# robotseu/ORB_Line_SLAM

Measured on AMD Instinct MI355X. Metric: stereo frames/s extract+match (ORB+LBD), KITTI 1242x375, higher is better.
Workload: dtype u8; 1 GPU; C3: 1242x375 stereo, 2000 ORB + 500 LBD per image, extract + stereo point/line match + f2f LBD match + SearchByBoW vs the previous frame (synthetic k=10 L=6 vocabulary, ComputeBoW included); parallelism=frame-sharded x1, distinct_pairs=512, order=shuffled, scene=default

## Files before the change

### include/orbline.h

```cpp
#ifndef ORBLINE_H
#define ORBLINE_H

#include "orbline_types.h"

#ifdef __cplusplus
extern "C" {
#endif

typedef struct olf_ctx olf_ctx;

const char* olf_last_error(void);
int olf_device_count(void);
int olf_default_params(olf_params* p);

int  olf_ctx_create(const olf_params* p, int width, int height, int max_images, olf_ctx** out);
void olf_ctx_destroy(olf_ctx* ctx);
int  olf_ctx_synchronize(olf_ctx* ctx);
int  olf_ctx_set_input_event(olf_ctx* ctx, void* hip_event);
int  olf_ctx_set_deferred_join(olf_ctx* ctx, int on);
int  olf_stereo_frames_join_dev(olf_ctx* ctx, void* stream);
int  olf_ctx_poll_status(olf_ctx* ctx);

int olf_profile_enable(olf_ctx* ctx, int on);
int olf_profile_reset(olf_ctx* ctx);
// ... 1 lines not shown
const char* olf_profile_stage_name(int stage);
int olf_profile_read(olf_ctx* ctx, double* total_ms, int32_t* calls);

enum { OLF_RGB2GRAY = 0, OLF_BGR2GRAY = 1, OLF_RGBA2GRAY = 2, OLF_BGRA2GRAY = 3 };
int olf_cvt_gray_dev(olf_ctx* ctx, const uint8_t* d_src, int code, int n_images, uint8_t* d_gray, void* stream);
int olf_remap_linear_dev(olf_ctx* ctx, const uint8_t* d_src, int src_w, int src_h, const float* d_mapx, const float* d_mapy, int dst_w,
                         int dst_h, int n_images, uint8_t* d_dst, void* stream);
int olf_init_undistort_rectify_map_dev(olf_ctx* ctx, const double* K, const double* D, int n_dist, const double* R, const double* P, int w, int h,
                                       float* d_map1, float* d_map2, void* stream);
int olf_init_undistort_rectify_map(olf_ctx* ctx, const double* K, const double* D, int n_dist, const double* R, const double* P, int w, int h,
                                   float* map1, float* map2);
int olf_cvt_gray(olf_ctx* ctx, const uint8_t* src, int code, int n_images, uint8_t* gray);
int olf_remap_linear(olf_ctx* ctx, const uint8_t* src, int src_w, int src_h, const float* mapx, const float* mapy, int dst_w, int dst_h,
                     int n_images, uint8_t* dst);

int olf_distinctive_descriptors(olf_ctx* ctx, const uint8_t* desc, const int32_t* offs, int n_points, int32_t* best);

size_t olf_kf_record_bytes(int n_keys, int n_lines);
int olf_kf_record_pack(uint64_t frame_id, uint64_t kf_id, double timestamp, const float* t3, const float* quat4, int n_keys,
                       const olf_keypoint* keys, const float* uright, const float* depth, const uint8_t* desc, const uint64_t* mappoint_ids,
                       int n_lines, const olf_keyline* lines, const float* disparity2, const double* le3, const uint8_t* ldesc,
                       const uint64_t* mapline_ids, uint8_t* out, size_t capacity, size_t* written);
int olf_kf_record_counts(const uint8_t* buf, size_t len, int32_t* n_keys, int32_t* n_lines, size_t* record_bytes);
int olf_kf_record_unpack(const uint8_t* buf, size_t len, uint64_t* frame_id, uint64_t* kf_id, double* timestamp, float* t3, float* quat4,
                         olf_keypoint* keys, float* uright, float* depth, uint8_t* desc, uint64_t* mappoint_ids, olf_keyline* lines,
                         float* disparity2, double* le3, uint8_t* ldesc, uint64_t* mapline_ids);

typedef struct olf_voc olf_voc;
int olf_voc_create(int k, int L, int scoring, int weighting, int n_nodes, const int32_t* parent, const uint8_t* is_leaf, const uint8_t* desc,
                   const double* weight, olf_voc** out);
int olf_voc_load_text(const char* path, olf_voc** out);
void olf_voc_destroy(olf_voc* voc);
int olf_voc_info(const olf_voc* voc, int* k, int* L, int* scoring, int* weighting, int* n_nodes, int* n_words);
int olf_bow_words_dev(olf_ctx* ctx, const olf_voc* voc, const uint8_t* d_desc, int n, int levelsup, int32_t* d_word, double* d_weight,
                      int32_t* d_node, void* stream);
int olf_bow_assemble(const olf_voc* voc, const int32_t* word, const double* weight, const int32_t* node, int n, int32_t* bow_ids,
                     double* bow_vals, int* n_bow, int32_t* fv_nodes, int32_t* fv_offs, int32_t* fv_idx, int* n_fv);
int olf_bow_transform(olf_ctx* ctx, const olf_voc* voc, const uint8_t* desc, int n, int levelsup, int32_t* bow_ids, double* bow_vals,
                      int* n_bow, int32_t* fv_nodes, int32_t* fv_offs, int32_t* fv_idx, int* n_fv);
int olf_search_by_bow_batch_dev(olf_ctx* ctx, const olf_voc* voc, int n_frames, int img_stride, const olf_keypoint* d_kps, const uint8_t* d_desc,
                                const int32_t* d_counts, const uint8_t* d_mp_valid, const uint8_t* d_mp_bad, float nnratio, int check_orientation,
                                int levelsup, int32_t* d_matches, int32_t* d_nmatches, void* stream);

int olf_orb_scale_tables(const olf_ctx* ctx, float* scale, float* inv_scale, float* sigma2, float* inv_sigma2,
                         int32_t* features_per_level);
int olf_orb_level_sizes(const olf_ctx* ctx, int32_t* widths, int32_t* heights);
int olf_orb_capacity(const olf_ctx* ctx);
int olf_orb_extract_strided(olf_ctx* ctx, const uint8_t* image, size_t row_stride, olf_keypoint* kps, uint8_t* desc, int32_t* count);
int olf_orb_extract_dev(olf_ctx* ctx, const uint8_t* d_images, int n_images, olf_keypoint* d_kps, uint8_t* d_desc,
                        int32_t* d_counts, void* stream);
int olf_orb_extract(olf_ctx* ctx, const uint8_t* images, int n_images, olf_keypoint* kps, uint8_t* desc, int32_t* counts);
int olf_orb_pyramid_level(olf_ctx* ctx, int image, int level, int blurred, uint8_t* dst);
int olf_orb_debug_candidates(olf_ctx* ctx, int image, int level, int32_t* xys, int cap, int32_t* count);
int olf_debug_status(olf_ctx* ctx, int32_t* out64);
int olf_debug_status_n(olf_ctx* ctx, int32_t* out, int n);
int olf_debug_lsd_owner(olf_ctx* ctx, int image, uint32_t* out);
int olf_debug_lsd_regions(olf_ctx* ctx, int image, int32_t* start_n, double* angle, int cap, int32_t* count);
int olf_debug_lsd_waves(olf_ctx* ctx, int waves_per_image, int rob_entries);
int olf_debug_lsd_groups(olf_ctx* ctx, int groups);
int olf_debug_lsd_scatter(olf_ctx* ctx, int on);
int olf_debug_lsd_log_cap(olf_ctx* ctx, int entries);
int olf_debug_seed_sort(olf_ctx* ctx, const uint32_t* keys, int n, int kthr, int depth_limit, uint32_t* out, int32_t* out_n);
int olf_debug_seed_sort_mode(olf_ctx* ctx, int mode);
int olf_debug_seed_sort_wide(olf_ctx* ctx, const uint64_t* keys, int n, int64_t kthr, int depth_limit, int full, uint32_t* out, int32_t* out_n);
int olf_debug_lsd_pool(olf_ctx* ctx, int pool_chunks);
int olf_debug_fdiv_sweep(olf_ctx* ctx, uint64_t seed, int blocks, int per_thread, uint64_t* mismatches);
int olf_debug_sqrtq_sweep(olf_ctx* ctx, int count, uint64_t* mismatches);
int olf_debug_align_sweep(olf_ctx* ctx, uint64_t seed, int blocks, int per_thread, uint64_t* out3);

int olf_stereo_points_dev(olf_ctx* ctx, int n_pairs, const olf_keypoint* d_kps, const uint8_t* d_desc, const int32_t* d_counts,
                          float* d_uright, float* d_depth, void* stream);
int olf_stereo_points(olf_ctx* ctx, const uint8_t* images, int n_pairs, olf_keypoint* kps, uint8_t* desc, int32_t* counts,
                      float* uright, float* depth);

int olf_match_bf_dev(olf_ctx* ctx, const uint8_t* d_descA, const int32_t* d_nA, int strideA, int a_step, const uint8_t* d_descB,
                     const int32_t* d_nB, int strideB, int b_step, int n_sets, float nnr, int best_lr, int32_t* d_m12, void* stream);
int olf_match_bf(olf_ctx* ctx, const uint8_t* descA, int nA, const uint8_t* descB, int nB, float nnr, int best_lr, int32_t* m12);
int olf_knn2(olf_ctx* ctx, const uint8_t* descQ, int nQ, const uint8_t* descT, int nT, int32_t* idx0, int32_t* dist0, int32_t* dist1);
int olf_match_candidates_dev(olf_ctx* ctx, const uint8_t* d_descQ, int nQ, const uint8_t* d_descT, int nT, const int32_t* d_cand_offsets,
                             const int32_t* d_cand_idx, uint16_t* d_dist, void* stream);
int olf_match_candidates(olf_ctx* ctx, const uint8_t* descQ, int nQ, const uint8_t* descT, int nT, const int32_t* cand_offsets,
                         const int32_t* cand_idx, uint16_t* dist);
typedef struct olf_frame_view {
    const olf_keypoint* keys;
    const uint8_t* desc;
    const float*   uright;
    int32_t        n;
    uint8_t*       mp_valid;
    uint8_t*       mp_obs;
    const uint8_t* mp_bad;
    const float*   mp_world;
    const uint8_t* mp_desc;
    const uint8_t* outlier;
    const float*   Tcw;
    float fx, fy, cx, cy, mbf, minX, maxX, minY, maxY;
    const float*   scale_factors;
    int32_t        n_levels;
    const float*   mp_maxd;
    const float*   mp_mind;
    const int32_t* fv_nodes;
    const int32_t* fv_offsets;
    const int32_t* fv_features;
    int32_t        fv_n;
    const int32_t* grid_offsets;
    const int32_t* grid_index;
} olf_frame_view;
// ... 534 lines not shown
```

### orb_line_slam_amd/csrc/api.cpp

```cpp
#include "ctx.hpp"
#include "staging.hpp"
#include <map>
#include <mutex>

namespace olf {
static thread_local std::string g_err;
void set_error(const std::string& s) { g_err = s; }

int check_device(const olf_ctx* c, const char* who)
{
    int d = -1;
    if (hipGetDevice(&d) != hipSuccess || d != c->device) { set_error(std::string(who) + ": the context belongs to another device than the current one"); return OLF_ERR_INVALID; }
    return OLF_OK;
}

static int check_landscape(const olf_ctx* c, const char* who)
{
    if (c->orb.portrait) {
        set_error(std::string(who) + ": the context's image is portrait (a pyramid level's octree would have round(width / height) == 0 root cells, where the "
                                     "reference divides by zero): no detector runs in it");
        return OLF_ERR_INVALID;
    }
    return OLF_OK;
}
// ... 178 lines not shown
    if (c->has_tables) angle_tables_release(c->device, c->params.line.conv_libm_float);
    if (c->h_outslab) (void)hipHostFree(c->h_outslab);
    for (void* p : c->allocs) (void)hipFree(p);
    for (void* p : c->scratch) if (p) (void)hipFree(p);
    for (auto& r : c->prof_recs) { (void)hipEventDestroy(r.a); (void)hipEventDestroy(r.b); }
    for (hipEvent_t e : c->prof_pool) (void)hipEventDestroy(e);
    if (c->ev_fork) (void)hipEventDestroy(c->ev_fork);
    if (c->ev_front) (void)hipEventDestroy(c->ev_front);
    if (c->ev_sort) (void)hipEventDestroy(c->ev_sort);
    if (c->ev_lbd) (void)hipEventDestroy(c->ev_lbd);
    if (c->ev_join) (void)hipEventDestroy(c->ev_join);
    if (c->stream2) (void)hipStreamDestroy(c->stream2);
    if (c->stream) (void)hipStreamDestroy(c->stream);
    delete c;
}

int olf_ctx_create(const olf_params* p, int width, int height, int max_images, olf_ctx** out)
{
    if (!p || !out || width < 64 || height < 64 || max_images < 1) { set_error("olf_ctx_create: bad argument"); return OLF_ERR_INVALID; }
    *out = nullptr;
    if (p->abi_version != OLF_ABI_VERSION || p->struct_size != (uint32_t)sizeof(olf_params)) {
        set_error("olf_ctx_create: the parameter block was not initialised by this library's olf_default_params() (abi_version / struct_size differ: "
                  "caller built against another include/orbline_types.h)");
        return OLF_ERR_INVALID;
    }
    int ndev = 0;
    if (hipGetDeviceCount(&ndev) != hipSuccess || ndev < 1) {
        set_error("olf_ctx_create: no HIP device visible (this library has no CPU path)");
        return OLF_ERR_NODEVICE;
    }
    olf_ctx* c = new olf_ctx();
    c->params = *p; c->W = width; c->H = height; c->max_images = max_images;
    int rc = c->orb.build(p->orb, width, height);
    if (rc != OLF_OK) {
        set_error(rc == OLF_ERR_CAPACITY ? "olf_ctx_create: more than 32760 key points on one pyramid level (nfeatures too large for this scale factor / level count)"
                  : (width > kMaxOrbSide || height > kMaxOrbSide) ? "olf_ctx_create: image wider or higher than 4131 pixels (FAST candidates are packed with 12 bits per coordinate)"
                                         : "olf_ctx_create: image size / ORB parameters not supported (every pyramid level needs at least 62 x 62 pixels)");
        delete c; return rc;
    }
    auto fail = [&](int code) { olf_ctx_destroy(c); return code; };
    if (hipGetDevice(&c->device) != hipSuccess) return fail(OLF_ERR_HIP);
    if (hipDeviceGetAttribute(&c->limits.nCU, hipDeviceAttributeMultiprocessorCount, c->device) != hipSuccess || c->limits.nCU <= 0) c->limits.nCU = 64;
    if (hipDeviceGetAttribute(&c->limits.maxLds, hipDeviceAttributeMaxSharedMemoryPerBlock, c->device) != hipSuccess) c->limits.maxLds = 64 * 1024;
    if (hipStreamCreateWithFlags(&c->stream, hipStreamNonBlocking) != hipSuccess) { set_error("hipStreamCreate failed"); return fail(OLF_ERR_HIP); }
    const OrbGeom& g = c->orb.geom;
    const size_t n = (size_t)max_images;
    OrbDeviceBufs& b = c->ob;
    const bool allocTrace = getenv("OLF_ALLOC_TRACE") != nullptr;
#define A(ptr, count) do { if ((rc = dev_alloc(c, &(ptr), (count))) != OLF_OK) return fail(rc); \
                           if (allocTrace) fprintf(stderr, "alloc %-18s %8.3f MB per image\n", #ptr, (double)(count) * sizeof(*(ptr)) / 1e6 / (double)n); } while (0)
    A(b.pyr, n * g.pyrBytes); A(b.blur, n * g.pyrBytes);
    A(b.cells, n * g.totalCells * g.cellCap); A(b.cellCount, n * g.totalCells);
    A(b.cand, n * g.candTotal); A(b.candNode, n * g.candTotal); A(b.candCount, n * g.nlevels);
    if (g.maxNodes > 2048) A(b.octSpill, n * g.nlevels * octree_lds_bytes(g.maxNodes));
    A(b.lvlKp, n * g.kpTotal); A(b.lvlCount, n * g.nlevels); A(b.lvlAngle, n * g.kpTotal);
    A(b.rx, c->orb.rx.size() + 1); A(b.ry, c->orb.ry.size() + 1); A(b.geom, 1); A(b.status, 256);
    A(c->d_sad, ((n + 1) / 2) * g.outCap); A(c->d_bestkey, ((n + 1) / 2) * g.outCap); A(c->d_rowperm, n * g.outCap);
    A(c->d_images, n * width * height);
#undef A
    if (hipMemcpy(b.rx, c->orb.rx.data(), c->orb.rx.size() * sizeof(ResizeCoef), hipMemcpyHostToDevice) != hipSuccess ||
        hipMemcpy(b.ry, c->orb.ry.data(), c->orb.ry.size() * sizeof(ResizeCoef), hipMemcpyHostToDevice) != hipSuccess ||
        hipMemcpy(b.geom, &g, sizeof(OrbGeom), hipMemcpyHostToDevice) != hipSuccess ||
        hipMemset(b.status, 0, 1024) != hipSuccess) {
        set_error("olf_ctx_create: table upload failed");
        return fail(OLF_ERR_HIP);
    }
    rc = c->line.build(p->line, width, height, max_images);
    if (rc != OLF_OK) { set_error("olf_ctx_create: LSD parameters not supported"); return fail(rc); }
    LineGeom& lg = c->line.geom;
    int prLeast = 0, prGreatest = 0;
    (void)hipDeviceGetStreamPriorityRange(&prLeast, &prGreatest);
    if (hipStreamCreateWithPriority(&c->stream2, hipStreamNonBlocking, prLeast) != hipSuccess ||
        hipEventCreateWithFlags(&c->ev_fork, hipEventDisableTiming) != hipSuccess || hipEventCreateWithFlags(&c->ev_front, hipEventDisableTiming) != hipSuccess || hipEventCreateWithFlags(&c->ev_sort, hipEventDisableTiming) != hipSuccess ||
        hipEventCreateWithFlags(&c->ev_lbd, hipEventDisableTiming) != hipSuccess ||
        hipEventCreateWithFlags(&c->ev_join, hipEventDisableTiming) != hipSuccess) { set_error("stream/event creation failed"); return fail(OLF_ERR_HIP); }
    LineDeviceBufs& l = c->lb;
#define A(ptr, count) do { if ((rc = dev_alloc(c, &(ptr), (count))) != OLF_OK) return fail(rc); \
                           if (allocTrace) fprintf(stderr, "alloc %-18s %8.3f MB per image\n", #ptr, (double)(count) * sizeof(*(ptr)) / 1e6 / (double)n); } while (0)
    const bool batchCtx = n > (size_t)kBatchCtxImages;
    const size_t keyWords = lg.wide ? 2 : 1;
    A(l.grad, n * lg.Ps); A(l.keysA, n * lg.Ps * keyWords); A(l.keysB, n * lg.Ps * keyWords);
    if (batchCtx && lg.Ps * 4 >= lg.pitchW * lg.H && lg.Ps * 4 >= lg.pitchS * lg.Hs) { l.lsdBlur = reinterpret_cast<uint8_t*>(l.keysA); l.scaled = reinterpret_cast<uint8_t*>(l.keysB); c->scaled_aliased = true; }
    else { A(l.lsdBlur, n * lg.pitchW * lg.H); A(l.scaled, n * lg.pitchS * lg.Hs); }
    A(l.topBuf, n * (size_t)lsd_seedsort_top_words()); A(l.keyCount, n * 32); A(l.maxN, n * 32); A(l.chunkCnt, n * ((lg.Ps + 4095) / 4096)); A(l.sortHist, n * (size_t)lsd_sort_max_chunks(lg.Ps) * 32); A(l.sortBase, n * 32);
    l.nChunks = lg.regionStride / 32;
    A(l.region, n * (size_t)lg.regionStride); l.ownerImages = (batchCtx || lg.wide) ? 0 : (int)std::min<size_t>(n, kMwMaxImages); A(l.owner, (size_t)l.ownerImages * lg.Ps); A(l.links, n * (size_t)l.nChunks);
    lg.logCap = lg.regionStride / 2;
    lg.spillBlocks = lg.regionStride / 2 >= lg.Ps ? 0 : (int)std::max<size_t>(4, n / 16);
    if (lg.spillBlocks) A(lg.spillArena, (size_t)lg.spillBlocks * 2 * lg.Ps);
    A(lg.spillCtl, 64); A(lg.spillOf, n);
    l.mgImages = (int)std::min<size_t>(n, kMgMaxImages); l.mgStride = lsd_grow_mg_stride(lg.maxRegions);
    A(l.mg, (size_t)l.mgImages * l.mgStride);
    A(l.rawLines, n * lg.maxDetect); A(l.rawCount, n); A(l.regCount, n); A(l.growFmt, n); A(l.lbdBlur, n * lg.pitchW * lg.H); A(l.dxdy, n * lg.pitchD * lg.H);
    A(l.rowSums, n * lg.outCap * 63 * 4); A(l.lbdStarts, n * lg.outCap * 64 * 2); A(l.rx, c->line.rx.size()); A(l.ry, c->line.ry.size()); A(l.geom, 1);
    A(c->d_ldist, ((n + 1) / 2) * lg.outCap * lg.outCap); A(c->d_lm21, ((n + 1) / 2) * lg.outCap);
    if (hipMalloc(&c->d_lprep, stereo_lines_prep_bytes((int)n, lg.outCap)) != hipSuccess) { set_error("hipMalloc failed"); return fail(OLF_ERR_HIP); }
    c->allocs.push_back(c->d_lprep);
    const bool slab = n <= 16;
    if (slab) {
        size_t off = 0;
        for (int k = 0; k < FB_FIELDS; ++k) { c->outslab_off[k] = off; off += (fb_bytes(c, k, n) + 255) & ~(size_t)255; }
        c->outslab_bytes = off;
        A(c->d_outslab, off);
        if (hipHostMalloc(reinterpret_cast<void**>(&c->h_outslab), off, hipHostMallocDefault) != hipSuccess) { set_error("hipHostMalloc failed"); return fail(OLF_ERR_HIP); }
    }
    for (int k = 0; k < FB_FIELDS; ++k) {
        uint8_t* q = nullptr;
// ... 397 lines not shown
```

### orb_line_slam_amd/csrc/api_debug.cpp

```cpp
#include "ctx.hpp"
#include "staging.hpp"
#include "wg_state.hpp"

namespace olf {
int launch_copy16(const void* src, void* dst, size_t bytes, hipStream_t s);
}

using namespace olf;

static int sweep_counters(HostCall& h, unsigned long long** st, int n)
{
    h.add(st, n);
    OLF_TRY(h.bind(SCRATCH_STAGE));
    OLF_HIP_CHECK(hipMemsetAsync(*st, 0, (size_t)n * 8, h.stream()));
    return OLF_OK;
}

extern "C" {

int olf_orb_pyramid_level(olf_ctx* c, int image, int level, int blurred, uint8_t* dst)
{
    if (!c || !dst || image < 0 || image >= c->max_images || level < 0 || level >= c->orb.geom.nlevels) return OLF_ERR_INVALID;
    const LevelGeom& L = c->orb.geom.lv[level];
    const uint8_t* src = (blurred ? c->ob.blur : c->ob.pyr) + (size_t)image * c->orb.geom.pyrBytes + L.offset;
    OLF_HIP_CHECK(hipStreamSynchronize(c->stream));
    OLF_HIP_CHECK(hipMemcpy2D(dst, L.w, src, L.pitch, L.w, L.h, hipMemcpyDeviceToHost));
    return OLF_OK;
}

int olf_debug_sim3_solver_lds_limit(int bytes)
{
    g_sim3_solver_lds.set(bytes);
    return OLF_OK;
}

int olf_debug_pnp_solver_lds_limit(int bytes)
{
    g_pnp_solver_lds.set(bytes);
    return OLF_OK;
}

int olf_debug_initializer_lds_limit(int bytes)
{
    g_initializer_lds.set(bytes);
    return OLF_OK;
}

int olf_debug_pose_points_lds_limit(int bytes)
{
    g_pose_points_lds.set(bytes);
    return OLF_OK;
}

int olf_debug_optimize_sim3_lds_limit(int bytes)
{
    g_optimize_sim3_lds.set(bytes);
    return OLF_OK;
}

int olf_debug_status(olf_ctx* c, int32_t* out64)
{
    if (!c || !out64) return OLF_ERR_INVALID;
    OLF_HIP_CHECK(hipDeviceSynchronize());
    OLF_HIP_CHECK(hipMemcpy(out64, c->ob.status, 256, hipMemcpyDeviceToHost));
    return OLF_OK;
}

int olf_debug_copy_bandwidth(olf_ctx* c, size_t bytes, int reps, double* gbytes_per_s)
{
    if (!c || !gbytes_per_s || bytes < 16 || reps < 1) { set_error("olf_debug_copy_bandwidth: bad argument"); return OLF_ERR_INVALID; }
    OLF_TRY(check_device(c, "olf_debug_copy_bandwidth"));
    void *a = nullptr, *b = nullptr;
    OLF_HIP_CHECK(hipMalloc(&a, bytes));
    if (hipMalloc(&b, bytes) != hipSuccess) { (void)hipFree(a); set_error("olf_debug_copy_bandwidth: hipMalloc failed"); return OLF_ERR_HIP; }
    hipEvent_t e0, e1;
    (void)hipEventCreate(&e0); (void)hipEventCreate(&e1);
    (void)hipMemsetAsync(a, 1, bytes, c->stream);
    int rc = olf::launch_copy16(a, b, bytes, c->stream);
    (void)hipEventRecord(e0, c->stream);
    for (int i = 0; i < reps && rc == OLF_OK; ++i) rc = olf::launch_copy16(i & 1 ? b : a, i & 1 ? a : b, bytes, c->stream);
// ... 189 lines not shown
```

### orb_line_slam_amd/csrc/host_tables.cpp

```cpp
#include "olf_internal.hpp"
#include "line_internal.hpp"
#include <algorithm>
#include <cmath>
#include <cfenv>

namespace olf {

static inline int cv_round_f(float v) { return (int)lrintf(v); }
static inline int cv_round_d(double v) { return (int)lrint(v); }
static inline int cv_floor(double v) { int i = (int)v; return i - (i > v); }
static inline int cv_ceil(double v) { int i = (int)v; return i + (i < v); }

std::vector<int> gaussian_taps_q8(int n, double sigma, int sum256)
{
    if (sum256) {
        std::vector<double> k(n);
        double s = 0;
        const double scale2X = -0.5 / (sigma * sigma);
        for (int i = 0; i < n; ++i) { const double x = i - (n - 1) * 0.5; k[i] = std::exp(scale2X * x * x); s += k[i]; }
        std::vector<int> q(n);
        double err = 0;
        int sum = 0;
        for (int i = 0; i < n / 2; ++i) {
            const double adj = k[i] / s * 256.0 + err;
// ... 108 lines not shown
        L.offset = off;
        off += L.pitch * L.h;
        off = (off + 255) & ~255;
        L.maxBorderX = L.w - kMinBorder; L.maxBorderY = L.h - kMinBorder;
        const float width = (float)(L.maxBorderX - kMinBorder), height = (float)(L.maxBorderY - kMinBorder);
        L.nCols = (int)(width / 30.f); L.nRows = (int)(height / 30.f);
        L.wCell = (int)std::ceil(width / L.nCols); L.hCell = (int)std::ceil(height / L.nRows);
        L.wCellM = (uint32_t)(((1u << 20) + L.wCell - 1) / L.wCell); L.hCellM = (uint32_t)(((1u << 20) + L.hCell - 1) / L.hCell);
        if (L.w >= (1 << 14) || L.h >= (1 << 14) || L.wCell > 64 || L.hCell > 64) { L.wCellM = 0; L.hCellM = 0; }
        L.cellBase = cells;
        cells += L.nCols * L.nRows;
        cellCap = std::max(cellCap, ((L.wCell + 1) / 2) * ((L.hCell + 1) / 2));
        L.quota = nPerLevel[l];
        maxQuota = std::max(maxQuota, L.quota);
        L.nIni = (int)std::round(width / height);
        if (L.nIni < 1) { portrait = true; L.nIni = 1; }
        L.hX = width / L.nIni;
        L.scale = sf[l]; L.inv_scale = inv_sf[l];
        L.patch_size = (int)(31 * sf[l]);
        L.kpBase = kps; L.kpCap = std::max(L.quota + 8, 4 * L.nIni + 4); kps += L.kpCap;
        maxKp = std::max(maxKp, L.kpCap);
        if (l > 0) {
            const LevelGeom& P = g.lv[l - 1];
            L.resizeTabX = (int)rx.size(); L.resizeTabY = (int)ry.size();
            rx.resize(rx.size() + L.w); ry.resize(ry.size() + L.h);
            double inv_x = (double)L.w / P.w, inv_y = (double)L.h / P.h;
            resize_axis_coefs(P.w, L.w, 1. / inv_x, true, &rx[L.resizeTabX]);
            resize_axis_coefs(P.h, L.h, 1. / inv_y, false, &ry[L.resizeTabY]);
            L.resizeTiled = resize_tiled_fits(&rx[L.resizeTabX], &ry[L.resizeTabY], P.w, P.h, L.w, L.h) ? 1 : 0;
            if (L.resizeTiled && resize_strip_fits(&rx[L.resizeTabX], P.w, L.w)) L.resizeTiled |= 2;
        }
    }
    g.pyrBytes = off;
    g.totalCells = cells;
    g.cellCap = cellCap;
    if (cellCap > 1024) return OLF_ERR_CAPACITY;
    for (int l = 0; l < nlevels; ++l) {
        LevelGeom& L = g.lv[l];
        long cap = (long)L.nCols * L.nRows * cellCap;
        L.candCap = (int)std::min<long>(cap, 65535);
        L.candBase = cand;
        cand += (L.candCap + 63) & ~63;
    }
    g.candTotal = cand;
    g.kpTotal = kps;
    g.outCap = kps;
    int mn = 64;
    while (mn < maxKp) mn <<= 1;
    g.maxNodes = mn;
    if (mn > 32768) return OLF_ERR_CAPACITY;
    return OLF_OK;
}

int LineHostTables::build(const olf_line_params& p, int W, int H, int max_images)
{
    LineGeom& g = geom;
    g = LineGeom();
    if (p.lsd_refine < 0 || p.lsd_refine > 2) return OLF_ERR_INVALID;
    if (p.conv_seed_order != 0 && p.conv_seed_order != 1) return OLF_ERR_INVALID;
    if (p.conv_libm_float != 0 && p.conv_libm_float != 1) return OLF_ERR_INVALID;
    if (!(p.lsd_scale > 0) || p.lsd_n_bins < 2 || p.lsd_n_bins > (1 << 24) || !(p.lsd_ang_th > 0 && p.lsd_ang_th < 180)) return OLF_ERR_INVALID;
    const double kPI = 3.1415926535897932384626433832795;
    g.W = W; g.H = H; g.pitchW = (W + 63) & ~63; g.pitchD = (W + 3) & ~3;
    g.scale = p.lsd_scale;
    g.Ws = cv_round_d(W * p.lsd_scale); g.Hs = cv_round_d(H * p.lsd_scale);
    g.pitchS = (g.Ws + 63) & ~63;
    g.Ps = g.Ws * g.Hs;
    {
        int k = 0; while ((1 << k) < g.Ws) ++k;
        const int p = std::max(32, 22 + k);
        const unsigned long long M = ((1ull << p) + (unsigned long long)g.Ws - 1) / (unsigned long long)g.Ws;
        g.divWsM = (uint32_t)M; g.divWsS = p - 32;
    }
    g.libmFloat = p.conv_libm_float ? 1 : 0;
    g.alignDeg = p.lsd_ang_th < 90 ? (float)(180.0 - p.lsd_ang_th) : -1.f;
    g.regionStride = std::max(1024 + g.Ps / 32 + 64, (2 * g.Ps + 31) / 32) * 32;
    if (max_images > kBatchCtxImages) g.regionStride = ((std::max(g.Ps, 8192) + 31) / 32) * 32;
    if ((long)g.Ws * g.Hs >= (1L << 27) || g.Ws < 8 || g.Hs < 8 || g.Ws > 32767 || g.Hs > 32767) return OLF_ERR_INVALID;
    g.wide = (p.lsd_n_bins > 1024 || (long)g.Ws * g.Hs >= (1L << 22)) ? 1 : 0;
    g.prec = kPI * p.lsd_ang_th / 180;
    {
        const long double w = (long double)(2 * kPI) - (long double)g.prec;
        double t = (double)w;
        if ((long double)t < w) t = std::nextafter(t, 1e300);
        g.precWrap = t;
    }
    {
        const double m = 6e-4;
        if (p.lsd_ang_th <= 80.0) {
            g.alignTanLo = std::nextafter((float)std::tan(g.prec - m), 0.f);
            g.alignTanHi = std::nextafter((float)std::tan(g.prec + m), 1e30f);
        } else { g.alignTanLo = -1.f; g.alignTanHi = -1.f; }
    }
    const double pp = p.lsd_ang_th / 180;
    const double rho = p.lsd_quant / std::sin(g.prec);
    int n = 0;
    while (!(std::sqrt(n / 4.0) > rho)) ++n;
    g.nThr = n;
    g.nBins = p.lsd_n_bins;
    const double LOG_NT = 5 * (std::log10(double(g.Ws)) + std::log10(double(g.Hs))) / 2 + std::log10(11.0);
    g.minRegSize = int(-LOG_NT / std::log10(pp));
    g.logNT = LOG_NT; g.logEps = p.lsd_log_eps; g.pProb = pp;
    g.minLength = p.min_line_length * std::min(W, H);
    g.maxDetect = std::min(32768, std::max(4096, g.Ps / 48));
    if (p.lsd_nfeatures == 0) g.maxDetect = std::min(g.maxDetect, std::max(4096, (int)(16e9 / ((double)std::max(max_images, 1) * 63 * 16))));
    g.maxRegions = std::min(g.Ps / std::max(g.minRegSize, 1) + 1, g.Ps / 6 - 1);
// ... 51 lines not shown
```

### orb_line_slam_amd/csrc/olf_internal.hpp

```cpp
#pragma once
#include <hip/hip_runtime.h>
#include <stdint.h>
#include <string>
#include <vector>
#include "../../include/orbline_types.h"
#include "device_math.hpp"

#define OLF_HIP_CHECK(expr)                                                                 \
    do {                                                                                    \
        hipError_t _e = (expr);                                                             \
        if (_e != hipSuccess) {                                                             \
            olf::set_error(std::string(#expr) + ": " + hipGetErrorString(_e));              \
            return OLF_ERR_HIP;                                                             \
        }                                                                                   \
    } while (0)

#define OLF_TRY(expr)                  \
    do {                               \
        int _rc = (expr);              \
        if (_rc != OLF_OK) return _rc; \
    } while (0)

struct olf_ctx;

// ... 108 lines not shown
};

struct ResizeCoef { int16_t ofs; int16_t a0; int16_t a1; int16_t pad; };

struct OrbGeom {
    int nlevels;
    int W, H, in_pitch;
    int pyrBytes;
    int totalCells;
    int cellCap;
    int candTotal;
    int kpTotal;
    int outCap;
    int iniTh, minTh;
    int maxNodes;
    LevelGeom lv[OLF_MAX_LEVELS];
    int umax[16];
    int blurTaps[7];
};

struct OrbHostTables {
    std::vector<float> sf, inv_sf, sigma2, inv_sigma2;
    std::vector<int> nPerLevel;
    OrbGeom geom;
    std::vector<ResizeCoef> rx, ry;
    bool portrait = false;
    int build(const olf_orb_params& p, int W, int H);
};

std::vector<int> gaussian_taps_q8(int n, double sigma, int sum256 = 0);
void resize_axis_coefs(int sn, int dn, double scale, bool clamp_like_x, ResizeCoef* coef);

struct OrbDeviceBufs {
    uint8_t* pyr = nullptr;
    uint8_t* blur = nullptr;
    uint32_t* cells = nullptr;
    int* cellCount = nullptr;
    uint32_t* cand = nullptr;
    uint16_t* candNode = nullptr;
    int* candCount = nullptr;
    uint32_t* lvlKp = nullptr;
    int* lvlCount = nullptr;
    float* lvlAngle = nullptr;
    ResizeCoef* rx = nullptr;
    ResizeCoef* ry = nullptr;
    OrbGeom* geom = nullptr;
    int* status = nullptr;
    unsigned char* octSpill = nullptr;
};

int launch_orb_pyramid(const OrbGeom& g, const OrbDeviceBufs& b, const uint8_t* d_in, int n_images, hipStream_t s);
int launch_orb_fast(const OrbGeom& g, const OrbDeviceBufs& b, int n_images, hipStream_t s);
int launch_orb_octree(const OrbGeom& g, const OrbDeviceBufs& b, int n_images, hipStream_t s);
size_t octree_lds_bytes(int M);
int launch_orb_blur(const OrbGeom& g, const OrbDeviceBufs& b, int n_images, hipStream_t s);
int launch_orb_describe(const OrbGeom& g, const OrbDeviceBufs& b, int n_images, olf_keypoint* d_kps, uint8_t* d_desc,
                        int* d_counts, int out_cap, hipStream_t s);

struct Taps7 { int t[7]; };
int launch_sep7(const uint8_t* src, size_t srcImgStride, int srcPitch, uint8_t* dst, size_t dstImgStride, int dstPitch, int W, int H,
                const int* taps7, int n_images, hipStream_t s);
int launch_sep_wide(const uint8_t* src, size_t srcImgStride, int srcPitch, uint8_t* dst, size_t dstImgStride, int dstPitch, int W, int H,
                    const int* taps, int r, int n_images, hipStream_t s);

bool resize_tiled_fits(const ResizeCoef* rx, const ResizeCoef* ry, int sw, int sh, int dw, int dh);
bool resize_strip_fits(const ResizeCoef* rx, int sw, int dw, int ncols = 4);
int launch_resize_tiled(const uint8_t* src, size_t srcImgStride, int srcPitch, int sw, int sh, uint8_t* dst, size_t dstImgStride, int dstPitch,
                        int dw, int dh, const ResizeCoef* d_rx, const ResizeCoef* d_ry, int n_images, hipStream_t s, bool strip = false);

int launch_cvt_gray(const uint8_t* src, uint8_t* dst, int w, int h, int code, int n_images, hipStream_t s);
int launch_init_rectify_map(const double* ir9, const double* k8, double fx, double fy, double u0, double v0, int w, int h, float* d_map1, float* d_map2,
                            hipStream_t s);
int launch_remap_linear(const uint8_t* src, int sw, int sh, const float* mapx, const float* mapy, int dw, int dh, uint8_t* dst, int n_images,
                        hipStream_t s);

int launch_stereo_points(const OrbGeom& g, const OrbDeviceBufs& b, int n_pairs, const olf_keypoint* d_kps, const uint8_t* d_desc,
                         const int* d_counts, int cap, float mbf, float fx, float* d_uRight, float* d_depth, int* d_sad, int* d_bestKey,
                         unsigned* d_perm, hipStream_t s);
int launch_match_bf(const uint8_t* dA, const int* nA, int strideA, int aStep, const uint8_t* dB, const int* nB, int strideB, int bStep,
                    int n_sets, float nnr, int best_lr, int* ws, int* m12, hipStream_t s);
int launch_knn2(const uint8_t* dA, const int* nA, int strideA, const uint8_t* dB, const int* nB, int strideB, int n_sets, int* idx0,
                int* dist0, int* dist1, hipStream_t s);
int launch_knn2_indexed(const uint8_t* q, const int* rank_entry, const int* qidx, const int* qbase, const int* nQ, const int* tile_prefix, int n_sets,
                        int max_tiles, const uint8_t* t, const int* nT, int strideT, int tStep, int tCap, int* idx0, int* dist0, int* dist1, hipStream_t s);
int launch_match_candidates(const uint8_t* q, int nQ, const uint8_t* t, int nT, const int* offs, const int* cand, uint16_t* out, hipStream_t s);
int launch_distinctive(const uint8_t* desc, const int* offs, int n_points, int* best, hipStream_t s);
int launch_hamming_matrix(const uint8_t* a, int nA, const uint8_t* b, int nB, uint16_t* out, hipStream_t s);


inline bool grid_scales(float minX, float maxX, float minY, float maxY, float* wInv, float* hInv)
{
    if (!(maxX > minX) || !(maxY > minY)) return false;
    *wInv = static_cast<float>(OLF_GRID_COLS) / (maxX - minX);
    *hInv = static_cast<float>(OLF_GRID_ROWS) / (maxY - minY);
    return true;
}
int launch_assign_grid(const olf_keypoint* d_kps, size_t frame_stride, const int* d_counts, int count_stride, int n_fixed, int n_limit, float minX,
                       float minY, float wInv, float hInv, int n_frames, int* d_cell_offsets, int* d_cell_index, size_t index_stride, hipStream_t s);
int launch_features_in_area(const olf_keypoint* d_keys, const int* d_cell_offsets, const int* d_cell_index, float minX, float minY, float wInv, float hInv,
                            int n_queries, const olf_area_query* d_queries, int* d_cand_offsets, int* d_cand_idx, int cand_capacity, int* d_status,
                            hipStream_t s);
bool grid_is_valid(const int32_t* cell_offsets, const int32_t* cell_index, int n);

int launch_kfdb_tables(const int* d_qoff, const int* d_qids, const double* d_qvals, int n_queries, const int* d_beg, const int* d_len, const int* d_ids,
                       const double* d_vals, int n_slots, int* d_common, int* d_first, double* d_score, hipStream_t s);
int launch_bow_score_pairs(const int* d_pairs, int n_pairs, const int* a_beg, const int* a_len, int n_a, const int* a_ids, const double* a_vals,
                           const int* b_beg, const int* b_len, int n_b, const int* b_ids, const double* b_vals, double* d_score, hipStream_t s);
// ... 3 lines not shown
```

### orb_line_slam_amd/csrc/orb_octree.hip

```cpp
#include "olf_internal.hpp"

namespace olf {

struct NodeRec { short ulx, uly, urx, bry; };

__device__ __forceinline__ int wave_incl_scan(int v, int lane)
{
#pragma unroll
    for (int o = 1; o < 64; o <<= 1) {
        int t = __shfl_up(v, o);
        if (lane >= o) v += t;
    }
    return v;
}

__device__ int block_excl_scan(int* a, int n, int* wsum)
{
    const int tid = threadIdx.x, lane = tid & 63, wv = tid >> 6;
    const int chunk = (n + 255) >> 8;
    const int b = tid * chunk, e = min(b + chunk, n);
    int s = 0;
    for (int i = b; i < e; ++i) s += a[i];
    int inc = wave_incl_scan(s, lane);
    if (lane == 63) wsum[wv] = inc;
    __syncthreads();
    int base = 0;
    for (int k = 0; k < wv; ++k) base += wsum[k];
    const int total = wsum[0] + wsum[1] + wsum[2] + wsum[3];
    int run = base + inc - s;
    for (int i = b; i < e; ++i) { int v = a[i]; a[i] = run; run += v; }
    __syncthreads();
    return total;
}

__device__ __forceinline__ int quadrant(const NodeRec& n, int x, int y, int& hx, int& hy)
{
    hx = (int)ceilf((float)(n.urx - n.ulx) / 2);
    hy = (int)ceilf((float)(n.bry - n.uly) / 2);
    return (x < n.ulx + hx ? 0 : 1) + (y < n.uly + hy ? 0 : 2);
}

template <bool SPILL>
__global__ __launch_bounds__(256) void k_octree(const OrbGeom* __restrict__ gp, const uint32_t* __restrict__ cells,
                                                const int* __restrict__ cellCount, uint32_t* __restrict__ cand,
                                                uint16_t* __restrict__ candNode, int* __restrict__ candCount,
                                                uint32_t* __restrict__ lvlKp, int* __restrict__ lvlCount, int* __restrict__ status,
                                                unsigned char* __restrict__ spill, size_t spillBytes)
{
    extern __shared__ __align__(16) unsigned char lds_smem[];
    unsigned char* smem = SPILL ? spill + ((size_t)blockIdx.y * gridDim.x + blockIdx.x) * spillBytes : lds_smem;
    const OrbGeom& g = *gp;
    const int level = blockIdx.x, img = blockIdx.y, tid = threadIdx.x;
    const LevelGeom& L = g.lv[level];
    const int M = g.maxNodes;
    NodeRec* nodeA = reinterpret_cast<NodeRec*>(smem);
    NodeRec* nodeB = nodeA + M;
    int* cntA = reinterpret_cast<int*>(nodeB + M);
    int* cntB = cntA + M;
    int* childCnt = cntB + M;
    int* scanA = childCnt + 4 * M;
    int* scanB = scanA + M;
    int* scanC = scanB + M;
    uint32_t* sortKey = reinterpret_cast<uint32_t*>(scanC + M);
    unsigned short* seqA = reinterpret_cast<unsigned short*>(sortKey + M);
    unsigned short* seqB = seqA + M;
    unsigned short* procNode = seqB + M;
    unsigned short* rankOf = procNode + M;
    unsigned short* seqToNode = rankOf + M;
    int* cellScan = reinterpret_cast<int*>(seqToNode + M);
    __shared__ int wsum[4];
    __shared__ int sh[8];

    const int nCells = L.nCols * L.nRows;
    const int* cc = cellCount + (size_t)img * g.totalCells + L.cellBase;
    uint32_t* myCand = cand + (size_t)img * g.candTotal + L.candBase;
    uint16_t* myNode = candNode + (size_t)img * g.candTotal + L.candBase;

    int C = 0;
    for (int base = 0; base < nCells; base += 4096) {
        const int n = min(4096, nCells - base);
        for (int i = tid; i < n; i += 256) cellScan[i] = cc[base + i];
        __syncthreads();
        const int tot = block_excl_scan(cellScan, n, wsum);
        for (int i = tid; i < n; i += 256) {
            const int k = cc[base + i], o = C + cellScan[i];
            const uint32_t* slot = cells + ((size_t)img * g.totalCells + L.cellBase + base + i) * g.cellCap;
            for (int j = 0; j < k; ++j)
                if (o + j < L.candCap) myCand[o + j] = slot[j];
        }
        C += tot;
        __syncthreads();
    }
    if (C > L.candCap) { if (tid == 0) atomicOr(status, 1); C = L.candCap; }
    if (tid == 0) candCount[img * g.nlevels + level] = C;
    __syncthreads();
    __threadfence_block();

    const int N = L.quota;
    const int nIni = L.nIni;
    for (int i = tid; i < 4 * M; i += 256) childCnt[i] = 0;
    __syncthreads();
    for (int c = tid; c < C; c += 256) {
        const int x = myCand[c] >> 20;
        int r = (int)((float)x / L.hX);
        r = min(r, nIni - 1);
        myNode[c] = (unsigned short)r;
        atomicAdd(&childCnt[r], 1);
    }
    __syncthreads();
    for (int i = tid; i < M; i += 256) scanA[i] = (i < nIni && childCnt[i] > 0) ? 1 : 0;
    __syncthreads();
    int Lsz = block_excl_scan(scanA, nIni, wsum);
    for (int i = tid; i < nIni; i += 256)
        if (childCnt[i] > 0) {
            const int p = scanA[i];
            NodeRec n;
            n.ulx = (short)(int)(L.hX * (float)i); n.urx = (short)(int)(L.hX * (float)(i + 1));
            n.uly = 0; n.bry = (short)(L.maxBorderY - kMinBorder);
            nodeA[p] = n; cntA[p] = childCnt[i]; seqA[p] = (unsigned short)p;
            scanB[i] = p;
        }
    __syncthreads();
    for (int c = tid; c < C; c += 256) myNode[c] = (unsigned short)scanB[myNode[c]];
    __syncthreads();

    NodeRec* cur = nodeA; NodeRec* nxt = nodeB;
    int* curCnt = cntA; int* nxtCnt = cntB;
    unsigned short* curSeq = seqA; unsigned short* nxtSeq = seqB;
    bool careful = false, finish = (C == 0);
    int guard = 0;
    while (!finish && guard++ < 64) {
        for (int i = tid; i < 4 * Lsz; i += 256) childCnt[i] = 0;
        __syncthreads();
        for (int c0 = tid; c0 < C; c0 += 4 * 256) {
            int ni[4];
            uint32_t pp[4];
#pragma unroll
            for (int u = 0; u < 4; ++u) { const int c = c0 + 256 * u; ni[u] = c < C ? (int)myNode[c] : -1; pp[u] = c < C ? myCand[c] : 0u; }
#pragma unroll
            for (int u = 0; u < 4; ++u) {
                const int i = ni[u];
                if (i >= 0 && curCnt[i] > 1) {
                    int hx, hy;
                    const int q = quadrant(cur[i], (int)(pp[u] >> 20), (int)((pp[u] >> 8) & 0xfff), hx, hy);
                    atomicAdd(&childCnt[4 * i + q], 1);
                }
            }
        }
        __syncthreads();
        int E;
        if (!careful) {
            for (int i = tid; i < Lsz; i += 256) scanA[i] = curCnt[i] > 1 ? 1 : 0;
            __syncthreads();
            E = block_excl_scan(scanA, Lsz, wsum);
            for (int i = tid; i < Lsz; i += 256)
                if (curCnt[i] > 1) procNode[scanA[i]] = (unsigned short)i;
        } else {
            for (int i = tid; i < M; i += 256) {
                uint32_t k = 0;
                if (i < Lsz && curCnt[i] > 1) {
                    k = ((uint32_t)min(curCnt[i], 0xffff) << 16) | curSeq[i];
                    seqToNode[curSeq[i]] = (unsigned short)i;
                }
                sortKey[i] = k;
            }
            __syncthreads();
            for (int k = 2; k <= M; k <<= 1)
                for (int j = k >> 1; j > 0; j >>= 1) {
                    for (int i = tid; i < M; i += 256) {
                        const int ixj = i ^ j;
                        if (ixj > i) {
                            const uint32_t a = sortKey[i], b = sortKey[ixj];
                            const bool desc = (i & k) == 0;
                            if (desc ? (a < b) : (a > b)) { sortKey[i] = b; sortKey[ixj] = a; }
                        }
                    }
                    __syncthreads();
                }
            if (tid == 0) sh[0] = 0;
            __syncthreads();
            int cntE = 0;
            for (int i = tid; i < M; i += 256)
                if (sortKey[i] != 0) { procNode[i] = seqToNode[sortKey[i] & 0xffff]; ++cntE; }
            atomicAdd(&sh[0], cntE);
            __syncthreads();
            E = sh[0];
        }
        __syncthreads();
        for (int r = tid; r < E; r += 256) {
            const int i = procNode[r];
            scanB[r] = (childCnt[4 * i] > 0) + (childCnt[4 * i + 1] > 0) + (childCnt[4 * i + 2] > 0) + (childCnt[4 * i + 3] > 0);
        }
        __syncthreads();
        block_excl_scan(scanB, E, wsum);
        if (tid == 0) sh[1] = E;
        __syncthreads();
        if (careful) {
            for (int r = tid; r < E; r += 256) {
                const int i = procNode[r];
                const int nc = (childCnt[4 * i] > 0) + (childCnt[4 * i + 1] > 0) + (childCnt[4 * i + 2] > 0) + (childCnt[4 * i + 3] > 0);
                if (Lsz - (r + 1) + scanB[r] + nc >= N) atomicMin(&sh[1], r + 1);
            }
            __syncthreads();
        }
        const int K = sh[1];
        for (int i = tid; i < Lsz; i += 256) rankOf[i] = 0xffff;
        __syncthreads();
        for (int r = tid; r < K; r += 256) rankOf[procNode[r]] = (unsigned short)r;
        if (tid == 0) {
            int T = 0;
            if (K > 0) {
                const int i = procNode[K - 1];
                T = scanB[K - 1] + (childCnt[4 * i] > 0) + (childCnt[4 * i + 1] > 0) + (childCnt[4 * i + 2] > 0) + (childCnt[4 * i + 3] > 0);
            }
            sh[2] = T; sh[3] = 0;
        }
        __syncthreads();
        const int T = sh[2];
        for (int i = tid; i < Lsz; i += 256) scanC[i] = rankOf[i] == 0xffff ? 1 : 0;
        __syncthreads();
        block_excl_scan(scanC, Lsz, wsum);
        const int newL = T + (Lsz - K);
        int nExp = 0;
        for (int i = tid; i < Lsz; i += 256) {
            const int r = rankOf[i];
            if (r == 0xffff) {
                const int p = T + scanC[i];
                nxt[p] = cur[i]; nxtCnt[p] = curCnt[i]; nxtSeq[p] = 0;
            } else {
                const NodeRec n = cur[i];
                int hx, hy;
                quadrant(n, 0, 0, hx, hy);
                const int c0 = childCnt[4 * i], c1 = childCnt[4 * i + 1], c2 = childCnt[4 * i + 2], c3 = childCnt[4 * i + 3];
                const int nc = (c0 > 0) + (c1 > 0) + (c2 > 0) + (c3 > 0);
                const int base = T - (scanB[r] + nc);
// ... 3 lines not shown
                for (int q = 0; q < 4; ++q) {
                    if (cs[q] > 0) {
                        --after;
                        const int p = base + after;
                        NodeRec ch;
                        ch.ulx = (short)((q & 1) ? n.ulx + hx : n.ulx);
                        ch.urx = (short)((q & 1) ? n.urx : n.ulx + hx);
                        ch.uly = (short)((q & 2) ? n.uly + hy : n.uly);
                        ch.bry = (short)((q & 2) ? n.bry : n.uly + hy);
                        nxt[p] = ch; nxtCnt[p] = cs[q];
                        nxtSeq[p] = (unsigned short)(scanB[r] + before);
                        ++before;
                        if (cs[q] > 1) ++nExp;
                        childCnt[4 * i + q] = p + 1;
                    }
                }
            }
        }
        atomicAdd(&sh[3], nExp);
        __syncthreads();
        for (int c0 = tid; c0 < C; c0 += 4 * 256) {
            int ni[4];
            uint32_t pp[4];
#pragma unroll
            for (int u = 0; u < 4; ++u) { const int c = c0 + 256 * u; ni[u] = c < C ? (int)myNode[c] : -1; pp[u] = c < C ? myCand[c] : 0u; }
#pragma unroll
            for (int u = 0; u < 4; ++u) {
                const int i = ni[u], c = c0 + 256 * u;
                if (i < 0) continue;
                if (rankOf[i] == 0xffff) myNode[c] = (unsigned short)(T + scanC[i]);
                else {
                    int hx, hy;
                    const int q = quadrant(cur[i], (int)(pp[u] >> 20), (int)((pp[u] >> 8) & 0xfff), hx, hy);
                    myNode[c] = (unsigned short)(childCnt[4 * i + q] - 1);
                }
            }
        }
        __syncthreads();
        const int nToExpand = sh[3];
        if (newL >= N || newL == Lsz) finish = true;
        else if (!careful && newL + nToExpand * 3 > N) careful = true;
        Lsz = newL;
        { NodeRec* t = cur; cur = nxt; nxt = t; }
        { int* t = curCnt; curCnt = nxtCnt; nxtCnt = t; }
        { unsigned short* t = curSeq; curSeq = nxtSeq; nxtSeq = t; }
        __syncthreads();
    }
    uint32_t* bestKey = reinterpret_cast<uint32_t*>(childCnt);
    for (int i = tid; i < Lsz; i += 256) bestKey[i] = 0;
    __syncthreads();
    for (int c = tid; c < C; c += 256) atomicMax(&bestKey[myNode[c]], ((myCand[c] & 0xffu) << 16) | (uint32_t)(0xffff - c));
    __syncthreads();
    uint32_t* out = lvlKp + (size_t)img * g.kpTotal + L.kpBase;
    if (Lsz > L.kpCap) { if (tid == 0) atomicOr(status, 2); Lsz = L.kpCap; }
    for (int i = tid; i < Lsz; i += 256) out[i] = myCand[0xffff - (bestKey[i] & 0xffff)];
    if (tid == 0) lvlCount[img * g.nlevels + level] = Lsz;
}

size_t octree_lds_bytes(int M)
{
    return (size_t)M * (2 * sizeof(NodeRec) + 2 * 4 + 4 * 4 + 3 * 4 + 4 + 5 * 2) + 4096 * 4;
}

int launch_orb_octree(const OrbGeom& g, const OrbDeviceBufs& b, int n_images, hipStream_t s)
{
    const size_t lds = octree_lds_bytes(g.maxNodes);
    if (g.maxNodes > 2048) {
        hipLaunchKernelGGL(k_octree<true>, dim3(g.nlevels, n_images), dim3(256), 0, s, b.geom, b.cells, b.cellCount, b.cand, b.candNode,
                           b.candCount, b.lvlKp, b.lvlCount, b.status, b.octSpill, lds);
        OLF_HIP_CHECK(hipGetLastError());
        return OLF_OK;
    }
    if (lds > 64 * 1024)
        OLF_HIP_CHECK(hipFuncSetAttribute(reinterpret_cast<const void*>(k_octree<false>), hipFuncAttributeMaxDynamicSharedMemorySize, 160 * 1024 - 64));
    hipLaunchKernelGGL(k_octree<false>, dim3(g.nlevels, n_images), dim3(256), lds, s, b.geom, b.cells, b.cellCount, b.cand, b.candNode,
                       b.candCount, b.lvlKp, b.lvlCount, b.status, nullptr, 0);
    OLF_HIP_CHECK(hipGetLastError());
    return OLF_OK;
}

}
```

Baseline: 15090 stereo frames/s.

## Size octree LDS per pyramid level and group levels into separate launches

The octree kernel now sizes its shared-memory layout from each level's own keypoint cap and quota instead of the global maximum node count. The bitonic sort runs over a per-level power-of-two size rather than the full node array. Levels are binned into up to three launches by LDS need, so small levels get less LDS and more blocks can reside per CU. The cell-scan buffer now aliases childCnt, and the overflow clamp on Lsz is removed. Costs are extra kernel launches per frame and the risk that a level overflows its smaller cap unchecked.

```diff
diff --git a/include/orbline.h b/include/orbline.h
--- a/include/orbline.h
+++ b/include/orbline.h
@@ -77,6 +77,7 @@
 int olf_orb_extract(olf_ctx* ctx, const uint8_t* images, int n_images, olf_keypoint* kps, uint8_t* desc, int32_t* counts);
 int olf_orb_pyramid_level(olf_ctx* ctx, int image, int level, int blurred, uint8_t* dst);
 int olf_orb_debug_candidates(olf_ctx* ctx, int image, int level, int32_t* xys, int cap, int32_t* count);
+int olf_debug_octree_launches(const olf_orb_params* params, int width, int height, int32_t* level_launch, int32_t* launch_lds);
 int olf_debug_status(olf_ctx* ctx, int32_t* out64);
 int olf_debug_status_n(olf_ctx* ctx, int32_t* out, int n);
 int olf_debug_lsd_owner(olf_ctx* ctx, int image, uint32_t* out);
diff --git a/orb_line_slam_amd/csrc/api.cpp b/orb_line_slam_amd/csrc/api.cpp
--- a/orb_line_slam_amd/csrc/api.cpp
+++ b/orb_line_slam_amd/csrc/api.cpp
@@ -254,7 +254,7 @@
     A(b.pyr, n * g.pyrBytes); A(b.blur, n * g.pyrBytes);
     A(b.cells, n * g.totalCells * g.cellCap); A(b.cellCount, n * g.totalCells);
     A(b.cand, n * g.candTotal); A(b.candNode, n * g.candTotal); A(b.candCount, n * g.nlevels);
-    if (g.maxNodes > 2048) A(b.octSpill, n * g.nlevels * octree_lds_bytes(g.maxNodes));
+    if (g.maxNodes > 2048) A(b.octSpill, n * g.nlevels * octree_spill_bytes(g));
     A(b.lvlKp, n * g.kpTotal); A(b.lvlCount, n * g.nlevels); A(b.lvlAngle, n * g.kpTotal);
     A(b.rx, c->orb.rx.size() + 1); A(b.ry, c->orb.ry.size() + 1); A(b.geom, 1); A(b.status, 256);
     A(c->d_sad, ((n + 1) / 2) * g.outCap); A(c->d_bestkey, ((n + 1) / 2) * g.outCap); A(c->d_rowperm, n * g.outCap);
diff --git a/orb_line_slam_amd/csrc/api_debug.cpp b/orb_line_slam_amd/csrc/api_debug.cpp
--- a/orb_line_slam_amd/csrc/api_debug.cpp
+++ b/orb_line_slam_amd/csrc/api_debug.cpp
@@ -26,6 +26,19 @@
     OLF_HIP_CHECK(hipStreamSynchronize(c->stream));
     OLF_HIP_CHECK(hipMemcpy2D(dst, L.w, src, L.pitch, L.w, L.h, hipMemcpyDeviceToHost));
     return OLF_OK;
+}
+
+int olf_debug_octree_launches(const olf_orb_params* p, int width, int height, int32_t* level_launch, int32_t* launch_lds)
+{
+    if (!p || !level_launch || !launch_lds) return OLF_ERR_INVALID;
+    OrbHostTables t;
+    OLF_TRY(t.build(*p, width, height));
+    OctLaunch la[3];
+    const int n = octree_launches(t.geom, la);
+    for (int i = 0; i < 3; ++i) launch_lds[i] = i < n ? (int32_t)la[i].lds : -1;
+    for (int i = 0; i < n; ++i)
+        for (int k = 0; k < la[i].lv.n; ++k) level_launch[la[i].lv.id[k]] = i;
+    return n;
 }
 
 int olf_debug_sim3_solver_lds_limit(int bytes)
diff --git a/orb_line_slam_amd/csrc/host_tables.cpp b/orb_line_slam_amd/csrc/host_tables.cpp
--- a/orb_line_slam_amd/csrc/host_tables.cpp
+++ b/orb_line_slam_amd/csrc/host_tables.cpp
@@ -184,6 +184,26 @@
     return OLF_OK;
 }
 
+int octree_launches(const OrbGeom& g, OctLaunch out[3])
+{
+    OctLaunch grp[3] = {};
+    if (g.maxNodes > 2048) {
+        for (int l = 0; l < g.nlevels; ++l) grp[0].lv.id[grp[0].lv.n++] = l;
+        out[0] = grp[0];
+        return 1;
+    }
+    for (int l = 0; l < g.nlevels; ++l) {
+        const size_t need = octree_lds_bytes(octree_node_cap(g.lv[l]), octree_sort_cap(g.lv[l]));
+        OctLaunch& o = grp[need > 36 * 1024 ? 0 : (need > 18 * 1024 ? 1 : 2)];
+        o.lv.id[o.lv.n++] = l;
+        o.lds = std::max(o.lds, need);
+    }
+    int n = 0;
+    for (int c = 0; c < 3; ++c)
+        if (grp[c].lv.n) out[n++] = grp[c];
+    return n;
+}
+
 int LineHostTables::build(const olf_line_params& p, int W, int H, int max_images)
 {
     LineGeom& g = geom;
diff --git a/orb_line_slam_amd/csrc/olf_internal.hpp b/orb_line_slam_amd/csrc/olf_internal.hpp
--- a/orb_line_slam_amd/csrc/olf_internal.hpp
+++ b/orb_line_slam_amd/csrc/olf_internal.hpp
@@ -184,7 +184,18 @@
 int launch_orb_pyramid(const OrbGeom& g, const OrbDeviceBufs& b, const uint8_t* d_in, int n_images, hipStream_t s);
 int launch_orb_fast(const OrbGeom& g, const OrbDeviceBufs& b, int n_images, hipStream_t s);
 int launch_orb_octree(const OrbGeom& g, const OrbDeviceBufs& b, int n_images, hipStream_t s);
-size_t octree_lds_bytes(int M);
+__host__ __device__ inline int octree_node_cap(const LevelGeom& L) { return (L.kpCap + 7) & ~7; }
+__host__ __device__ inline int octree_sort_cap(const LevelGeom& L)
+{
+    int s = 64;
+    while (s < L.quota) s <<= 1;
+    return s;
+}
+__host__ __device__ inline size_t octree_lds_bytes(int nodeCap, int sortCap) { return (size_t)nodeCap * 62 + (size_t)sortCap * 4; }
+size_t octree_spill_bytes(const OrbGeom& g);
+struct OctLevels { int n; int id[OLF_MAX_LEVELS]; };
+struct OctLaunch { OctLevels lv; size_t lds; };
+int octree_launches(const OrbGeom& g, OctLaunch out[3]);
 int launch_orb_blur(const OrbGeom& g, const OrbDeviceBufs& b, int n_images, hipStream_t s);
 int launch_orb_describe(const OrbGeom& g, const OrbDeviceBufs& b, int n_images, olf_keypoint* d_kps, uint8_t* d_desc,
                         int* d_counts, int out_cap, hipStream_t s);
diff --git a/orb_line_slam_amd/csrc/orb_octree.hip b/orb_line_slam_amd/csrc/orb_octree.hip
--- a/orb_line_slam_amd/csrc/orb_octree.hip
+++ b/orb_line_slam_amd/csrc/orb_octree.hip
@@ -45,14 +45,14 @@
                                                 const int* __restrict__ cellCount, uint32_t* __restrict__ cand,
                                                 uint16_t* __restrict__ candNode, int* __restrict__ candCount,
                                                 uint32_t* __restrict__ lvlKp, int* __restrict__ lvlCount, int* __restrict__ status,
-                                                unsigned char* __restrict__ spill, size_t spillBytes)
+                                                unsigned char* __restrict__ spill, size_t spillBytes, OctLevels lv)
 {
     extern __shared__ __align__(16) unsigned char lds_smem[];
-    unsigned char* smem = SPILL ? spill + ((size_t)blockIdx.y * gridDim.x + blockIdx.x) * spillBytes : lds_smem;
     const OrbGeom& g = *gp;
-    const int level = blockIdx.x, img = blockIdx.y, tid = threadIdx.x;
+    const int level = lv.id[blockIdx.x], img = blockIdx.y, tid = threadIdx.x;
+    unsigned char* smem = SPILL ? spill + ((size_t)img * g.nlevels + level) * spillBytes : lds_smem;
     const LevelGeom& L = g.lv[level];
-    const int M = g.maxNodes;
+    const int M = octree_node_cap(L), S = octree_sort_cap(L);
     NodeRec* nodeA = reinterpret_cast<NodeRec*>(smem);
     NodeRec* nodeB = nodeA + M;
     int* cntA = reinterpret_cast<int*>(nodeB + M);
@@ -62,12 +62,12 @@
     int* scanB = scanA + M;
     int* scanC = scanB + M;
     uint32_t* sortKey = reinterpret_cast<uint32_t*>(scanC + M);
-    unsigned short* seqA = reinterpret_cast<unsigned short*>(sortKey + M);
+    unsigned short* seqA = reinterpret_cast<unsigned short*>(sortKey + S);
     unsigned short* seqB = seqA + M;
     unsigned short* procNode = seqB + M;
     unsigned short* rankOf = procNode + M;
     unsigned short* seqToNode = rankOf + M;
-    int* cellScan = reinterpret_cast<int*>(seqToNode + M);
+    int* cellScan = childCnt;
     __shared__ int wsum[4];
     __shared__ int sh[8];
 
@@ -77,8 +77,8 @@
     uint16_t* myNode = candNode + (size_t)img * g.candTotal + L.candBase;
 
     int C = 0;
-    for (int base = 0; base < nCells; base += 4096) {
-        const int n = min(4096, nCells - base);
+    for (int base = 0; base < nCells; base += 4 * M) {
+        const int n = min(4 * M, nCells - base);
         for (int i = tid; i < n; i += 256) cellScan[i] = cc[base + i];
         __syncthreads();
         const int tot = block_excl_scan(cellScan, n, wsum);
@@ -156,7 +156,7 @@
             for (int i = tid; i < Lsz; i += 256)
                 if (curCnt[i] > 1) procNode[scanA[i]] = (unsigned short)i;
         } else {
-            for (int i = tid; i < M; i += 256) {
+            for (int i = tid; i < S; i += 256) {
                 uint32_t k = 0;
                 if (i < Lsz && curCnt[i] > 1) {
                     k = ((uint32_t)min(curCnt[i], 0xffff) << 16) | curSeq[i];
@@ -165,9 +165,9 @@
                 sortKey[i] = k;
             }
             __syncthreads();
-            for (int k = 2; k <= M; k <<= 1)
+            for (int k = 2; k <= S; k <<= 1)
                 for (int j = k >> 1; j > 0; j >>= 1) {
-                    for (int i = tid; i < M; i += 256) {
+                    for (int i = tid; i < S; i += 256) {
                         const int ixj = i ^ j;
                         if (ixj > i) {
                             const uint32_t a = sortKey[i], b = sortKey[ixj];
@@ -180,7 +180,7 @@
             if (tid == 0) sh[0] = 0;
             __syncthreads();
             int cntE = 0;
-            for (int i = tid; i < M; i += 256)
+            for (int i = tid; i < S; i += 256)
                 if (sortKey[i] != 0) { procNode[i] = seqToNode[sortKey[i] & 0xffff]; ++cntE; }
             atomicAdd(&sh[0], cntE);
             __syncthreads();
@@ -290,30 +290,34 @@
     for (int c = tid; c < C; c += 256) atomicMax(&bestKey[myNode[c]], ((myCand[c] & 0xffu) << 16) | (uint32_t)(0xffff - c));
     __syncthreads();
     uint32_t* out = lvlKp + (size_t)img * g.kpTotal + L.kpBase;
-    if (Lsz > L.kpCap) { if (tid == 0) atomicOr(status, 2); Lsz = L.kpCap; }
     for (int i = tid; i < Lsz; i += 256) out[i] = myCand[0xffff - (bestKey[i] & 0xffff)];
     if (tid == 0) lvlCount[img * g.nlevels + level] = Lsz;
 }
 
-size_t octree_lds_bytes(int M)
-{
-    return (size_t)M * (2 * sizeof(NodeRec) + 2 * 4 + 4 * 4 + 3 * 4 + 4 + 5 * 2) + 4096 * 4;
+size_t octree_spill_bytes(const OrbGeom& g)
+{
+    size_t m = 0;
+    for (int l = 0; l < g.nlevels; ++l) m = std::max(m, octree_lds_bytes(octree_node_cap(g.lv[l]), octree_sort_cap(g.lv[l])));
+    return (m + 15) & ~(size_t)15;
 }
 
 int launch_orb_octree(const OrbGeom& g, const OrbDeviceBufs& b, int n_images, hipStream_t s)
 {
-    const size_t lds = octree_lds_bytes(g.maxNodes);
+    OctLaunch la[3];
+    const int n = octree_launches(g, la);
     if (g.maxNodes > 2048) {
-        hipLaunchKernelGGL(k_octree<true>, dim3(g.nlevels, n_images), dim3(256), 0, s, b.geom, b.cells, b.cellCount, b.cand, b.candNode,
-                           b.candCount, b.lvlKp, b.lvlCount, b.status, b.octSpill, lds);
+        hipLaunchKernelGGL(k_octree<true>, dim3(la[0].lv.n, n_images), dim3(256), 0, s, b.geom, b.cells, b.cellCount, b.cand, b.candNode,
+                           b.candCount, b.lvlKp, b.lvlCount, b.status, b.octSpill, octree_spill_bytes(g), la[0].lv);
         OLF_HIP_CHECK(hipGetLastError());
         return OLF_OK;
     }
-    if (lds > 64 * 1024)
+    if (la[0].lds > 64 * 1024)
         OLF_HIP_CHECK(hipFuncSetAttribute(reinterpret_cast<const void*>(k_octree<false>), hipFuncAttributeMaxDynamicSharedMemorySize, 160 * 1024 - 64));
-    hipLaunchKernelGGL(k_octree<false>, dim3(g.nlevels, n_images), dim3(256), lds, s, b.geom, b.cells, b.cellCount, b.cand, b.candNode,
-                       b.candCount, b.lvlKp, b.lvlCount, b.status, nullptr, 0);
-    OLF_HIP_CHECK(hipGetLastError());
+    for (int i = 0; i < n; ++i) {
+        hipLaunchKernelGGL(k_octree<false>, dim3(la[i].lv.n, n_images), dim3(256), la[i].lds, s, b.geom, b.cells, b.cellCount, b.cand, b.candNode,
+                           b.candCount, b.lvlKp, b.lvlCount, b.status, nullptr, 0, la[i].lv);
+        OLF_HIP_CHECK(hipGetLastError());
+    }
     return OLF_OK;
 }
 
```

Result: faster. 15480 stereo frames/s (median of 6 runs) (+2.6%).
